# myscience/open-genie

Measured on NVIDIA H100. Metric: videotokenizer_train_step_frames_per_sec, higher is better.
Workload: dtype bf16

## Files before the change

### include/opengenie_b200.h

```cpp
#ifndef OPENGENIE_B200_H_
#define OPENGENIE_B200_H_

#include <stddef.h>
#include <stdint.h>

#ifdef __cplusplus
extern "C" {
#endif

typedef enum og_status {
  OG_OK = 0,
  OG_ERR_INVALID_ARGUMENT = -1,
  OG_ERR_UNSUPPORTED_SHAPE = -2,
  OG_ERR_CUDA = -3,
} og_status;

typedef void* og_stream_t;

const char* og_last_error(void);
int og_abi_version(void);
int og_compiled_sm(void);
uint64_t og_launch_count(void);


int og_conv3d_fwd(const void* x0, int c0, int kt, int kh, int kw, int pt, int ph, int pw, const void* x1, int c1,
                  const void* w, int ldw, const float* bias0, const float* bias1, const void* residual, void* out,
                  int out_f32, int N, int T, int H, int W, int cout, void* workspace, size_t workspace_bytes,
                  double* gn_sums, og_stream_t stream);

int og_conv3d_dgrad(const void* dy, int cout, int w_rows, const void* w, int ldw, int k_off, int kt, int kh, int kw,
                    int pt, int ph, int pw, void* dx, int dx_f32, int N, int T, int H, int W, int cin,
                    void* workspace, size_t workspace_bytes, og_stream_t stream);

int og_conv3d_wgrad(const void* dy, int cout, const void* x, int cin, float* dw, int64_t ld_dw, int kt, int kh,
                    int kw, int pt, int ph, int pw, int N, int T, int H, int W, void* workspace,
                    size_t workspace_bytes, og_stream_t stream);
int og_conv3d_wgrad_bias(const void* dy, int cout, const void* x, int cin, float* dw, int64_t ld_dw, int kt, int kh,
                         int kw, int pt, int ph, int pw, int N, int T, int H, int W, float* dbias, int n_bias,
                         void* workspace, size_t workspace_bytes, og_stream_t stream);

int og_conv3d_strided_fwd(const void* x, int cin, int kt, int kh, int kw, int st, int sh, int sw, int pt, int ph, int pw,
                          const void* w, int ldw, const float* bias, void* out, int out_f32, int N, int T, int H, int W,
                          int cout, og_stream_t stream);
int og_conv3d_strided_dgrad(const void* dy, int cout, int w_rows, const void* w, int ldw, int kt, int kh, int kw, int st,
                            int sh, int sw, int pt, int ph, int pw, void* dx, int N, int T, int H, int W, int cin,
                            og_stream_t stream);
int og_conv3d_strided_wgrad(const void* dy, int cout, const void* x, int cin, float* dw, int64_t ld_dw, int kt, int kh,
                            int kw, int st, int sh, int sw, int pt, int ph, int pw, int N, int T, int H, int W,
                            void* workspace, size_t workspace_bytes, og_stream_t stream);


int og_gn_stats(const void* x, int N, int64_t V, int C, int G, double* sums, og_stream_t stream);

int og_gn_finalize(const double* sums, int N, int C, int G, int64_t V, float eps, const float* gamma,
                   const float* beta, const float* cond_scale, const float* cond_shift, float* A, float* B,
                   float* mean_rstd, og_stream_t stream);

int og_affine_act_fwd(const void* x, const float* A, const float* B, void* y, int N, int64_t V, int C, int act,
                      og_stream_t stream);

int og_affine_act_bwd_reduce(const void* dy, const void* x, const float* A, const float* B, int act, float* S,
                             int N, int64_t V, int C, void* workspace, size_t workspace_bytes, og_stream_t stream);

int og_gn_bwd_finalize(const float* S, const float* mean_rstd, const float* gamma, const float* beta,
                       const float* cond_scale, int N, int C, int G, int64_t V, float* Q, float* R, float* dgamma,
                       float* dbeta, float* dcond_scale, float* dcond_shift, og_stream_t stream);

int og_affine_act_bwd_apply(const void* dy, const void* x, const float* A, const float* B, const float* Q,
                            const float* R, const void* add, void* dx, int act, int N, int64_t V, int C,
                            og_stream_t stream);

int og_adagn_cond_fwd(const float* cond, int N, int64_t V, int D, const float* w_scale, const float* b_scale,
                      const float* w_shift, const float* b_shift, int C, float* cbar, float* scale, float* shift,
                      og_stream_t stream);
int og_adagn_cond_bwd(const float* dscale, const float* dshift, const float* cbar, const float* w_scale,
                      const float* w_shift, int N, int64_t V, int D, int C, float* dw_scale, float* db_scale,
                      float* dw_shift, float* db_shift, float* dcond, og_stream_t stream);

int og_gn_act_fwd(const void* x, const double* sums, const float* gamma, const float* beta, const float* cond_scale,
                  const float* cond_shift, float eps, int G, int act, void* y, float* A, float* B, float* mean_rstd,
                  int N, int64_t V, int C, og_stream_t stream);
int og_gn_act_bwd(const void* dy, const void* x, const float* A, const float* B, const float* S,
                  const float* mean_rstd, const float* gamma, const float* beta, const float* cond_scale, int G, int act,
                  const void* add, void* dx, float* dgamma, float* dbeta, float* dcond_scale, float* dcond_shift,
                  float* dx_colsum, int N, int64_t V, int C, void* workspace, size_t workspace_bytes,
                  og_stream_t stream);


int og_ncdhw_f32_to_ndhwc(const float* x, void* y, int y_f32, int N, int C, int64_t V, og_stream_t stream);
int og_ndhwc_to_ncdhw_f32(const void* x, int x_f32, float* y, int N, int C, int64_t V, og_stream_t stream);

int og_pixel_shuffle3d(const void* x, void* y, int inverse, int N, int T, int H, int W, int c, int p, int q, int r,
                       og_stream_t stream);

int og_blurpool3d(const void* x, void* y, float* scratch, int backward, int N, int T, int H, int W, int cin, int cout,
                  int k, int st, int sh, int sw, og_stream_t stream);

int og_blurpool2d(const void* x, void* y, float* scratch, int backward, int N, int H, int W, int cin, int cout, int k,
                  int sh, int sw, int pad, og_stream_t stream);

int og_mse_fwd(const float* rec_ndhwc, const float* tgt_ncdhw, int N, int C, int64_t V, float* loss_sum,
               og_stream_t stream);
int og_mse_bwd(const float* rec_ndhwc, const float* tgt_ncdhw, const float* gscale, int N, int C, int cpad,
               int64_t V, void* drec, og_stream_t stream);

int og_maxpool2x2(const void* x, void* y, int N, int H, int W, int C, og_stream_t stream);
int og_sqdiff_sum(const void* a, const void* b, int64_t n, float* out, og_stream_t stream);

int og_colsum(const void* x, int64_t rows, int C, int ld, float* out, og_stream_t stream);
int og_pad_channels(const void* x, int x_f32, void* y, int64_t rows, int cs, int cd, og_stream_t stream);

int og_sub_rows(const void* a, const void* b, void* out, int64_t n, og_stream_t stream);

int og_copy_rows_to_bf16(const void* src, int src_f32, int64_t src_ld, void* dst, int64_t dst_ld, int64_t rows,
                         int cols, og_stream_t stream);

int og_frames_u8_to_video(const uint8_t* frames, int bgr, void* out, int out_kind, int cpad, int N, int T, int H, int W,
                          og_stream_t stream);

size_t og_lfq_workspace_bytes(int64_t ntok, int D);

int og_lfq_fwd(const float* x, int ldx, int64_t ntok, int D, float beta, int training, float w_commit,
               float w_entropy, float w_div, float* out_f32, void* out_bf16, int ld_bf16, int64_t* idx, float* loss,
               void* workspace, og_stream_t stream);

int og_lfq_bwd(const float* x, int ldx, int64_t ntok, int D, float beta, float w_commit, float w_entropy,
               const float* gloss, const float* dout, int ld_dout, float* dx_f32, void* dx_bf16, int ld_dx,
               void* workspace, og_stream_t stream);


int og_rope_table(const float* freq, int npos, int C, float* table, og_stream_t stream);
int og_rope_ln_fwd(const void* x, const float* freq, const float* gamma, const float* beta, float eps, void* y,
                   int64_t rows, int C, int64_t pos_div, int pos_mod, const float* cos_sin, og_stream_t stream);
int og_rope_ln_bwd(const void* x, const float* freq, const float* gamma, float eps, const void* g0, const void* g1,
                   const void* g2, const void* add, void* dx, float* dgamma, float* dbeta, int64_t rows, int C,
                   int64_t pos_div, int pos_mod, const float* cos_sin, og_stream_t stream);

int og_flash_attn_fwd(const void* q, const void* k, const void* v, void* out, const void* residual, void* out_res,
                      float* lse, int nseq, int S, int C, int n_head, float scale, og_stream_t stream);
int og_flash_attn_bwd(const void* q, const void* k, const void* v, const void* out, const void* dout,
                      const float* lse, float* delta_ws, void* dq, void* dk, void* dv, int nseq, int S, int C,
                      int n_head, float scale, og_stream_t stream);

int og_temporal_attn_fwd(const void* q, const void* k, const void* v, const void* residual, void* out, int B, int T,
                         int64_t P, int C, int n_head, float scale, int kv_bcast, og_stream_t stream);
int og_temporal_attn_bwd(const void* q, const void* k, const void* v, const void* dout, void* dq, void* dk, void* dv,
                         float* dk_bcast, float* dv_bcast, int B, int T, int64_t P, int C, int n_head, float scale,
                         int kv_bcast, og_stream_t stream);

int og_temporal_attn_long_fwd(const void* q, const void* k, const void* v, void* out, const void* residual,
                              void* out_res, float* lse, int B, int T, int64_t P, int C, int n_head, float scale,
                              int kv_bcast, og_stream_t stream);
int og_temporal_attn_long_bwd(const void* q, const void* k, const void* v, const void* out, const void* dout,
                              const float* lse, float* delta_ws, void* dq, void* dk, void* dv, float* dk_bcast,
                              float* dv_bcast, int B, int T, int64_t P, int C, int n_head, float scale, int kv_bcast,
                              og_stream_t stream);


int og_embed_add_fwd(const int64_t* tok, const int64_t* act, const float* tok_w, const float* act_w, void* out,
                     int64_t rows, int64_t rows_per_act, int C, int tok_vocab, int act_vocab, og_stream_t stream);
int og_embed_add_bwd(const int64_t* tok, const int64_t* act, const void* dy, float* d_tok_w, float* d_act_w,
                     int64_t rows, int64_t rows_per_act, int C, int tok_vocab, int act_vocab, og_stream_t stream);

int og_masked_ce_fwd(const void* logits, const int64_t* target, const uint8_t* mask, int64_t rows, int V,
                     float* row_lse, float* stats, og_stream_t stream);
int og_masked_ce_bwd(const void* logits, const int64_t* target, const uint8_t* mask, const float* row_lse,
                     const float* stats, const float* gloss, void* dlogits, int64_t rows, int V, og_stream_t stream);

int og_softmax_cdf(const void* logits, int logits_f32, int64_t rows, int V, float inv_temp, float* cdf,
                   float* row_stats, og_stream_t stream);
int og_maskgit_sample(const float* cdf, const void* logits, int logits_f32, float inv_temp, const float* row_stats,
                      const float* uniforms, const int* schedule, int steps, int B, int P, int V, int64_t* code,
                      uint8_t* mask, og_stream_t stream);

typedef struct og_adamw_tensor {
  float* p;
  const float* g;
  float* m;
  float* v;
  void* p_bf16;
  int64_t n;
  int64_t row_len;
  int64_t dst_ld;
} og_adamw_tensor;

int og_adamw_chunk_elems(void);
int og_adamw_step(const og_adamw_tensor* table_dev, const int* chunk_tensor_dev, const int* chunk_index_dev,
                  int num_chunks, float lr, float beta1, float beta2, float eps, float weight_decay, int step,
                  const int* step_dev, const float* lr_dev, const float* grad_scale_dev, og_stream_t stream);
int og_adamw_tick(int* step_dev, og_stream_t stream);

#ifdef __cplusplus
// ... 4 lines not shown
```

### open_genie_b200/csrc/conv3d_wgrad.cu

```cuda
#include "og_host.cuh"
#include "og_ptx.cuh"

namespace og {
extern std::atomic<uint64_t> g_launches;

static constexpr int kWThreads = 384;
static constexpr int kVox = 64;
static constexpr int kPanelBytes = kVox * 128;
static constexpr int kTileM = 128;
static constexpr int kTileN = 256;
static constexpr int kWABytes = 2 * kPanelBytes;
static constexpr int kWBBytes = 4 * kPanelBytes;
static constexpr int kWStages = 4;
static constexpr int kSlotFloats = kTileM * kTileN;

struct WgradParams {
  int kt, kh, kw, pt, ph, pw;
  int sx_t, sx_h, sx_w;
  int bw_log2, bh_log2, bt_log2, bn_log2;
  int tiles_w, tiles_h, tiles_t;
  int num_ksteps;
  int cin, cout;
  int ncols;
  int col_tiles;
  long long units;
  int ctas;
  int granule;
  int period;
  float* dw;
  long long ld_dw;
  int vec_ok;
  float* dbias;
  int n_bias;
  float* ws;
};

__host__ __device__ __forceinline__ long long share_begin(const WgradParams& p, int b) {
  return (long long)b * (p.units / p.granule) / p.ctas * p.granule;
}

template <bool kOnes>
__device__ __forceinline__ void wgrad_mma_steps(float (&acc)[128], float (&accb)[8], int nsteps, const uint8_t* smem_a,
                                                const uint8_t* smem_b, uint32_t ones_addr, uint64_t* full,
                                                uint64_t* empty, int& s, uint32_t& ph, int lane) {
  int prev = -1;
  for (int i = 0; i < nsteps; ++i) {
    mbar_wait(&full[s], ph);
    const uint32_t a_addr = smem_u32(smem_a + s * kWABytes);
    const uint32_t b_addr = smem_u32(smem_b + s * kWBBytes);
    wgmma_fence();
#pragma unroll
    for (int k = 0; k < kVox / 16; ++k)
      wgmma_ss<256, 1, 1>(acc, gmma_desc_sw128(a_addr + k * 2048, kPanelBytes, 1024),
                          gmma_desc_sw128(b_addr + k * 2048, kPanelBytes, 1024), (i | k) != 0);
    if constexpr (kOnes) {
#pragma unroll
      for (int k = 0; k < kVox / 16; ++k)
        wgmma_ss<16, 1, 1>(accb, gmma_desc_sw128(a_addr + k * 2048, kPanelBytes, 1024),
                           gmma_desc_sw128(ones_addr, kPanelBytes, 1024), (i | k) != 0);
    }
    wgmma_commit();
    wgmma_wait<1>();
    if (prev >= 0 && lane == 0) mbar_arrive(&empty[prev]);
    prev = s;
    if (++s == kWStages) {
      s = 0;
      ph ^= 1;
    }
  }
  wgmma_wait<0>();
  if (lane == 0) mbar_arrive(&empty[prev]);
}

template <bool kBias>
__global__ void __launch_bounds__(kWThreads, 1)
    og_conv_wgrad_kernel(const __grid_constant__ CUtensorMap mapDY, const __grid_constant__ CUtensorMap mapX,
                         const WgradParams p) {
  extern __shared__ uint8_t smem_raw[];
  uint8_t* smem = reinterpret_cast<uint8_t*>((reinterpret_cast<uintptr_t>(smem_raw) + 1023) & ~uintptr_t(1023));
  uint8_t* smem_a = smem;
  uint8_t* smem_b = smem + kWStages * kWABytes;
  uint8_t* smem_ones = smem_b + kWStages * kWBBytes;
  uint64_t* full = reinterpret_cast<uint64_t*>(smem_ones + 2048);
  uint64_t* empty = full + kWStages;

  const int warp = warp_idx_uniform();
  const int lane = threadIdx.x & 31;
  const long long u_begin = share_begin(p, blockIdx.x), u_end = share_begin(p, blockIdx.x + 1);

  if (warp == 0 && lane == 0) {
    tma_prefetch_desc(&mapDY);
    tma_prefetch_desc(&mapX);
    for (int s = 0; s < kWStages; ++s) {
      mbar_init(&full[s], 1);
      mbar_init(&empty[s], 8);
    }
    fence_mbar_init();
  }
  if (kBias) {
    for (int i = threadIdx.x; i < 2048 / 4; i += kWThreads) reinterpret_cast<uint32_t*>(smem_ones)[i] = 0x3F803F80u;
    fence_proxy_async_smem();
  }
  __syncthreads();

  if (warp == 0) {
    int s = 0;
    uint32_t ph = 0;
    const int per_sample = p.tiles_w * p.tiles_h * p.tiles_t;
    long long clock = 0;
    for (long long u = u_begin; u < u_end;) {
      const int tile = (int)(u / p.num_ksteps);
      const int k0 = (int)(u - (long long)tile * p.num_ksteps);
      const int k1 = (int)min((long long)p.num_ksteps, u_end - (long long)tile * p.num_ksteps);
      u += k1 - k0;
      const int co0 = (tile / p.col_tiles) * kTileM;
      const int c0 = (tile % p.col_tiles) * kTileN;
      const int npan = min(4, (p.ncols - c0) / 64);
      int pci[4], off_w[4], off_h[4], off_t[4];
#pragma unroll
      for (int j = 0; j < 4; ++j) {
        const int c = c0 + 64 * (j < npan ? j : 0);
        const int tap = c / p.cin;
        pci[j] = c - tap * p.cin;
        off_t[j] = tap / (p.kh * p.kw) - p.pt;
        off_h[j] = (tap / p.kw) % p.kh - p.ph;
        off_w[j] = tap % p.kw - p.pw;
      }
      const uint32_t tx_bytes = (uint32_t)(kWABytes + npan * kPanelBytes);
      int ks = k0 + (int)((clock - k0 % p.period + p.period) % p.period);
      if (ks >= k1) ks = k0;
      clock += k1 - k0;
      int tn, tw, th, tt;
      auto decode = [&](int k) {
        tn = k / per_sample;
        int r = k - tn * per_sample;
        tw = r % p.tiles_w;
        r /= p.tiles_w;
        th = r % p.tiles_h;
        tt = r / p.tiles_h;
      };
      decode(ks);
      for (int i = k0; i < k1; ++i) {
        const int n = tn << p.bn_log2, w0 = tw << p.bw_log2, h0 = th << p.bh_log2, t0 = tt << p.bt_log2;
        mbar_wait(&empty[s], ph ^ 1);
        if (elect_one()) {
          mbar_expect_tx(&full[s], tx_bytes);
          uint8_t* a = smem_a + s * kWABytes;
          tma_load_5d(a, &mapDY, &full[s], co0, w0, h0, t0, n);
          tma_load_5d(a + kPanelBytes, &mapDY, &full[s], co0 + 64, w0, h0, t0, n);
          uint8_t* b = smem_b + s * kWBBytes;
          for (int j = 0; j < npan; ++j)
            tma_load_5d(b + j * kPanelBytes, &mapX, &full[s], pci[j], w0 * p.sx_w + off_w[j], h0 * p.sx_h + off_h[j],
                        t0 * p.sx_t + off_t[j], n);
        }
        __syncwarp();
        if (++s == kWStages) {
          s = 0;
          ph ^= 1;
        }
        if (++ks == k1) {
          ks = k0;
          decode(ks);
        } else if (++tw == p.tiles_w) {
          tw = 0;
          if (++th == p.tiles_h) {
            th = 0;
            if (++tt == p.tiles_t) {
              tt = 0;
              ++tn;
            }
          }
        }
      }
    }
    __syncwarp();
  } else if (warp >= 4) {
    const int wg = (warp >> 2) - 1;
    const int q = warp & 3;
    const uint32_t ones_addr = smem_u32(smem_ones);
    const uint8_t* a_wg = smem_a + wg * kPanelBytes;
    float acc[128], accb[8];
    int s = 0;
    uint32_t ph = 0;
    for (long long u = u_begin; u < u_end;) {
      const bool first = u == u_begin;
      const int tile = (int)(u / p.num_ksteps);
      const int k0 = (int)(u - (long long)tile * p.num_ksteps);
      const int k1 = (int)min((long long)p.num_ksteps, u_end - (long long)tile * p.num_ksteps);
      u += k1 - k0;
      const int co0 = (tile / p.col_tiles) * kTileM;
      const int c0 = (tile % p.col_tiles) * kTileN;
      const bool bias_tile = kBias && c0 == 0;
      if (bias_tile)
        wgrad_mma_steps<true>(acc, accb, k1 - k0, a_wg, smem_b, ones_addr, full, empty, s, ph, lane);
      else
        wgrad_mma_steps<false>(acc, accb, k1 - k0, a_wg, smem_b, ones_addr, full, empty, s, ph, lane);
      reg_fence(acc);
      reg_fence(accb);
      const bool whole = k0 == 0 && k1 == p.num_ksteps;
      const int slot = 2 * blockIdx.x + (first ? 0 : 1);
      const int c_lane = 2 * (lane & 3);
#pragma unroll
      for (int rr = 0; rr < 2; ++rr) {
        const int r = wg * 64 + q * 16 + (lane >> 2) + rr * 8;
        const int co = co0 + r;
        if (whole) {
          if (co >= p.cout) continue;
          float* row = p.dw + (long long)co * p.ld_dw + c0 + c_lane;
#pragma unroll
          for (int j = 0; j < 32; ++j) {
            if (c0 + 8 * j + c_lane >= p.ncols) continue;
            const float v0 = acc[4 * j + 2 * rr], v1 = acc[4 * j + 2 * rr + 1];
            if (p.vec_ok) {
              float2* d = reinterpret_cast<float2*>(row + 8 * j);
              const float2 o = *d;
              *d = make_float2(o.x + v0, o.y + v1);
            } else {
              row[8 * j] += v0;
              row[8 * j + 1] += v1;
            }
          }
          if (bias_tile && (lane & 3) == 0 && co < p.n_bias) p.dbias[co] += accb[2 * rr];
        } else {
          float* sl = p.ws + ((long long)slot * kTileM + r) * kTileN + c_lane;
#pragma unroll
          for (int j = 0; j < 32; ++j)
            *reinterpret_cast<float2*>(sl + 8 * j) = make_float2(acc[4 * j + 2 * rr], acc[4 * j + 2 * rr + 1]);
          if (bias_tile && (lane & 3) == 0)
            p.ws[(long long)2 * p.ctas * kSlotFloats + (long long)slot * kTileM + r] = accb[2 * rr];
        }
      }
    }
  }
}

__global__ void __launch_bounds__(256) og_wgrad_fixup_kernel(const WgradParams p) {
  const int b = blockIdx.y;
  const long long ub = share_begin(p, b + 1);
  const int tile = (int)(ub / p.num_ksteps);
  const long long t0 = (long long)tile * p.num_ksteps, t1 = t0 + p.num_ksteps;
  if (ub == t0 || share_begin(p, b) > t0) return;
  const int co0 = (tile / p.col_tiles) * kTileM, c0 = (tile % p.col_tiles) * kTileN;
  const int e = (blockIdx.x * 256 + threadIdx.x) * 4;
  const int r = e / kTileN, c = e % kTileN;
  float4 sum = make_float4(0.f, 0.f, 0.f, 0.f);
  float sumb = 0.f;
  const bool bias = p.dbias && c0 == 0 && blockIdx.x == 0 && threadIdx.x < kTileM;
  for (int sh = b; sh < p.ctas; ++sh) {
    const long long sb = share_begin(p, sh);
    if (sb >= t1) break;
    const int slot = 2 * sh + (sb >= t0 ? 0 : 1);
    const float4 v = __ldcg(reinterpret_cast<const float4*>(p.ws + (long long)slot * kSlotFloats + e));
    sum.x += v.x;
    sum.y += v.y;
    sum.z += v.z;
    sum.w += v.w;
    if (bias) sumb += __ldcg(p.ws + (long long)2 * p.ctas * kSlotFloats + (long long)slot * kTileM + threadIdx.x);
  }
  if (co0 + r < p.cout && c0 + c < p.ncols) {
    float* d = p.dw + (long long)(co0 + r) * p.ld_dw + c0 + c;
    d[0] += sum.x;
    d[1] += sum.y;
    d[2] += sum.z;
    d[3] += sum.w;
  }
  if (bias && co0 + (int)threadIdx.x < p.n_bias) p.dbias[co0 + threadIdx.x] += sumb;
}

}

static int launch_wgrad(const void* dy, int cout, const void* x, int cin, float* dw, int64_t ld_dw, int kt, int kh, int kw,
                        int pt, int ph, int pw, int N, int T, int H, int W, int Ti, int Hi, int Wi, int st, int sh, int sw,
                        void* workspace, size_t workspace_bytes, og_stream_t stream, float* dbias = nullptr,
                        int n_bias = 0) {
  using namespace og;
  OG_REQUIRE(dy && x && dw, "conv3d_wgrad: null pointer");
  OG_REQUIRE(!dbias || (n_bias > 0 && n_bias <= cout), "conv3d_wgrad: n_bias=%d must be in 1..cout", n_bias);
  OG_REQUIRE(cin > 0 && cin % 64 == 0, "conv3d_wgrad: cin=%d must be a multiple of 64", cin);
  OG_REQUIRE(cout > 0 && cout % 8 == 0, "conv3d_wgrad: cout=%d must be a multiple of 8 (TMA row stride)", cout);
  OG_REQUIRE(kt >= 1 && kh >= 1 && kw >= 1 && pt >= 0 && ph >= 0 && pw >= 0 && pt < kt && ph < kh && pw < kw,
             "conv3d_wgrad: bad kernel/padding");
  OG_REQUIRE(st >= 1 && sh >= 1 && sw >= 1 && st <= 8 && sh <= 8 && sw <= 8, "conv3d_wgrad: bad stride");
  int bw, bh, bt, bn;
  choose_voxel_box(kVox, N, T, H, W, &bw, &bh, &bt, &bn);
  WgradParams p;
  memset(&p, 0, sizeof(p));
  p.kt = kt; p.kh = kh; p.kw = kw; p.pt = pt; p.ph = ph; p.pw = pw;
  p.sx_t = st; p.sx_h = sh; p.sx_w = sw;
  p.bw_log2 = ilog2(bw); p.bh_log2 = ilog2(bh); p.bt_log2 = ilog2(bt); p.bn_log2 = ilog2(bn);
  p.tiles_w = (W + bw - 1) / bw; p.tiles_h = (H + bh - 1) / bh; p.tiles_t = (T + bt - 1) / bt;
  p.num_ksteps = ((N + bn - 1) / bn) * p.tiles_w * p.tiles_h * p.tiles_t;
  p.cin = cin; p.cout = cout; p.dw = dw; p.ld_dw = ld_dw;
  p.ncols = kt * kh * kw * cin;
  p.col_tiles = (p.ncols + kTileN - 1) / kTileN;
  const long long tiles = (long long)((cout + kTileM - 1) / kTileM) * p.col_tiles;
  p.units = tiles * p.num_ksteps;
  const int sms = num_sms();
  p.ctas = (int)std::min<long long>(sms, std::max<long long>(1, p.units / 4));
  p.granule = 1;
  const size_t slot_bytes = (size_t)(kSlotFloats + (dbias ? kTileM : 0)) * sizeof(float);
  const long long fit = workspace ? (long long)(workspace_bytes / (2 * slot_bytes)) : 0;
  if (fit < p.ctas) {
    if (fit > tiles) {
      p.ctas = (int)fit;
    } else {
      p.granule = p.num_ksteps;
      p.ctas = (int)std::min<long long>(sms, tiles);
    }
  }
  p.period = (int)std::min<long long>(p.num_ksteps, (p.units + p.ctas - 1) / p.ctas);
  p.ws = reinterpret_cast<float*>(workspace);
  p.vec_ok = (ld_dw % 2 == 0) && ((reinterpret_cast<uintptr_t>(dw) & 7) == 0);
  p.dbias = dbias;
  p.n_bias = n_bias;
  const size_t smem_bytes = (size_t)kWStages * (kWABytes + kWBBytes) + 2048  + 1024 + 512;

  CUtensorMap mapDY, mapX;
  {
    uint64_t dims[5] = {(uint64_t)cout, (uint64_t)W, (uint64_t)H, (uint64_t)T, (uint64_t)N};
    uint64_t str[4] = {(uint64_t)cout * 2, (uint64_t)W * cout * 2, (uint64_t)H * W * cout * 2,
                       (uint64_t)T * H * W * cout * 2};
    uint32_t box[5] = {64, (uint32_t)bw, (uint32_t)bh, (uint32_t)bt, (uint32_t)bn};
    int r = make_tmap_bf16(&mapDY, dy, 5, dims, str, box);
    if (r != OG_OK) return r;
  }
  {
    uint64_t dims[5] = {(uint64_t)cin, (uint64_t)Wi, (uint64_t)Hi, (uint64_t)Ti, (uint64_t)N};
    uint64_t str[4] = {(uint64_t)cin * 2, (uint64_t)Wi * cin * 2, (uint64_t)Hi * Wi * cin * 2,
                       (uint64_t)Ti * Hi * Wi * cin * 2};
    uint32_t box[5] = {64, (uint32_t)(bw * sw), (uint32_t)(bh * sh), (uint32_t)(bt * st), (uint32_t)bn};
    uint32_t es[5] = {1, (uint32_t)sw, (uint32_t)sh, (uint32_t)st, 1};
    OG_REQUIRE(box[1] <= 256 && box[2] <= 256 && box[3] <= 256, "conv3d_wgrad: strided box exceeds the TMA limit");
    int r = make_tmap_bf16(&mapX, x, 5, dims, str, box, es);
    if (r != OG_OK) return r;
  }
  static bool attr_set = false;
  if (!attr_set) {
    OG_CHECK_CUDA(cudaFuncSetAttribute(og_conv_wgrad_kernel<false>, cudaFuncAttributeMaxDynamicSharedMemorySize,
                                       (int)smem_bytes));
    OG_CHECK_CUDA(cudaFuncSetAttribute(og_conv_wgrad_kernel<true>, cudaFuncAttributeMaxDynamicSharedMemorySize,
                                       (int)smem_bytes));
    attr_set = true;
  }
  if (dbias)
    og_conv_wgrad_kernel<true><<<p.ctas, kWThreads, smem_bytes, (cudaStream_t)stream>>>(mapDY, mapX, p);
  else
    og_conv_wgrad_kernel<false><<<p.ctas, kWThreads, smem_bytes, (cudaStream_t)stream>>>(mapDY, mapX, p);
  OG_CHECK_CUDA(cudaGetLastError());
  g_launches.fetch_add(1);
  if (p.granule == 1 && p.ctas > 1) {
    og_wgrad_fixup_kernel<<<dim3(kSlotFloats / 1024, p.ctas - 1), 256, 0, (cudaStream_t)stream>>>(p);
    OG_CHECK_CUDA(cudaGetLastError());
    g_launches.fetch_add(1);
  }
  return OG_OK;
}

extern "C" int og_conv3d_wgrad(const void* dy, int cout, const void* x, int cin, float* dw, int64_t ld_dw, int kt,
                               int kh, int kw, int pt, int ph, int pw, int N, int T, int H, int W, void* workspace,
                               size_t workspace_bytes, og_stream_t stream) {
  return launch_wgrad(dy, cout, x, cin, dw, ld_dw, kt, kh, kw, pt, ph, pw, N, T, H, W, T, H, W, 1, 1, 1, workspace,
                      workspace_bytes, stream);
}

extern "C" int og_conv3d_wgrad_bias(const void* dy, int cout, const void* x, int cin, float* dw, int64_t ld_dw, int kt,
                                    int kh, int kw, int pt, int ph, int pw, int N, int T, int H, int W, float* dbias,
                                    int n_bias, void* workspace, size_t workspace_bytes, og_stream_t stream) {
  if (!dbias) {
    og::set_error("conv3d_wgrad_bias: dbias is NULL");
    return OG_ERR_INVALID_ARGUMENT;
  }
  return launch_wgrad(dy, cout, x, cin, dw, ld_dw, kt, kh, kw, pt, ph, pw, N, T, H, W, T, H, W, 1, 1, 1, workspace,
                      workspace_bytes, stream, dbias, n_bias);
}

extern "C" int og_conv3d_strided_wgrad(const void* dy, int cout, const void* x, int cin, float* dw, int64_t ld_dw, int kt,
                                       int kh, int kw, int st, int sh, int sw, int pt, int ph, int pw, int N, int T, int H,
                                       int W, void* workspace, size_t workspace_bytes, og_stream_t stream) {
  const int To = (T + pt - kt) / st + 1, Ho = (H + 2 * ph - kh) / sh + 1, Wo = (W + 2 * pw - kw) / sw + 1;
  if (To < 1 || Ho < 1 || Wo < 1) {
    og::set_error("conv3d_strided_wgrad: empty output");
    return OG_ERR_INVALID_ARGUMENT;
  }
  return launch_wgrad(dy, cout, x, cin, dw, ld_dw, kt, kh, kw, pt, ph, pw, N, To, Ho, Wo, T, H, W, st, sh, sw, workspace,
                      workspace_bytes, stream);
}
```

### open_genie_b200/ops.py

```python
from __future__ import annotations

import ctypes
from typing import Optional, Tuple

import torch
from torch import Tensor

from . import _lib

bf16 = torch.bfloat16
f32 = torch.float32


def _stream() -> int:
    return torch.cuda.current_stream().cuda_stream


def _in_backward() -> bool:
    return torch._C._current_graph_task_id() != -1


class ZeroArena:

    SEGMENT = 256 << 20
# ... 976 lines not shown
    return y5.permute(0, 2, 3, 4, 1).reshape(rows, N)


class _EmbedAddFn(torch.autograd.Function):

    @staticmethod
    def forward(ctx, tokens, act_id, tok_w, act_w):
        _require_cuda(tok_w, 'embedding weight')
        if tokens.dim() != 4:
            raise ValueError(f'embed_add: tokens must be (B, T, H, W), got {tuple(tokens.shape)}')
        if tuple(act_id.shape) != tuple(tokens.shape[:2]):
            raise ValueError(f'embed_add: act_id shape {tuple(act_id.shape)} does not match the (B, T) = '
                             f'{tuple(tokens.shape[:2])} of the tokens (one action per token frame)')
        B, T, H, W = tokens.shape
        C = tok_w.shape[1]
        tok = tokens.detach().to(torch.int64).contiguous()
        act = act_id.detach().to(torch.int64).contiguous()
        out = torch.empty((B, T, H, W, C), dtype=bf16, device=tok_w.device)
        _lib.call('og_embed_add_fwd', tok.data_ptr(), act.data_ptr(), tok_w.data_ptr(), act_w.data_ptr(), out.data_ptr(),
                  B * T * H * W, H * W, C, tok_w.shape[0], act_w.shape[0], _stream())
        ctx.save_for_backward(tok, act)
        ctx.shapes = (tok_w.shape, act_w.shape, H * W)
        return out

    @staticmethod
    def backward(ctx, dy):
        tok, act = ctx.saved_tensors
        ts, as_, hw = ctx.shapes
        dy = _rows_bf16(dy)
        dtw = _zeros(ts, f32, dy.device)
        daw = _zeros(as_, f32, dy.device)
        _lib.call('og_embed_add_bwd', tok.data_ptr(), act.data_ptr(), dy.data_ptr(), dtw.data_ptr(), daw.data_ptr(),
                  tok.numel(), hw, ts[1], ts[0], as_[0], _stream())
        return None, None, dtw, daw


def embed_add(tokens, act_id, tok_w, act_w):
    return _EmbedAddFn.apply(tokens, act_id, tok_w, act_w)


class _MaskedCeFn(torch.autograd.Function):

    @staticmethod
    def forward(ctx, logits2d, target, mask):
        rows, V = logits2d.shape
        lg = logits2d if (logits2d.dtype == bf16 and logits2d.is_contiguous()) else logits2d.to(bf16).contiguous()
        tgt = target.detach().reshape(-1).to(torch.int64).contiguous()
        msk = mask.detach().reshape(-1).to(torch.uint8).contiguous()
        row_lse = torch.empty(rows, dtype=f32, device=lg.device)
        stats = torch.zeros(2, dtype=f32, device=lg.device)
        _lib.call('og_masked_ce_fwd', lg.data_ptr(), tgt.data_ptr(), msk.data_ptr(), rows, V, row_lse.data_ptr(),
                  stats.data_ptr(), _stream())
        ctx.save_for_backward(lg, tgt, msk, row_lse, stats)
        return stats[0] / stats[1]

    @staticmethod
    def backward(ctx, g):
        lg, tgt, msk, row_lse, stats = ctx.saved_tensors
        gs = g.detach().to(f32).contiguous()
        dl = torch.empty_like(lg)
        _lib.call('og_masked_ce_bwd', lg.data_ptr(), tgt.data_ptr(), msk.data_ptr(), row_lse.data_ptr(), stats.data_ptr(),
                  gs.data_ptr(), dl.data_ptr(), lg.shape[0], lg.shape[1], _stream())
        return dl, None, None


def masked_cross_entropy(logits2d, target, mask):
    return _MaskedCeFn.apply(logits2d, target, mask)


def maskgit_sample(logits_last: Tensor, uniforms: Tensor, schedule: Tensor, temp: float = 1.0, masked_tok: int = 0
                   ) -> Tensor:
    _require_cuda(logits_last, 'logits')
    b, h, w, V = logits_last.shape
    P = h * w
    lg = logits_last.detach()
    if lg.dtype not in (bf16, f32) or not lg.is_contiguous():
        lg = lg.float().contiguous()
    dev = lg.device
    s = _stream()
    cdf = torch.empty((b * P, V), dtype=f32, device=dev)
    row_stats = torch.empty((b * P, 2), dtype=f32, device=dev)
    lg_f32, inv_temp = int(lg.dtype == f32), 1.0 / float(temp)
    _lib.call('og_softmax_cdf', lg.data_ptr(), lg_f32, b * P, V, inv_temp, cdf.data_ptr(), row_stats.data_ptr(), s)
    steps = int(schedule.numel())
    u = uniforms.detach().to(device=dev, dtype=f32).reshape(steps, b * P).contiguous()
    sch = schedule.detach().to(device=dev, dtype=torch.int32).contiguous()
    code = torch.full((b, P), int(masked_tok), dtype=torch.int64, device=dev)
    mask = torch.ones((b, P), dtype=torch.uint8, device=dev)
    _lib.call('og_maskgit_sample', cdf.data_ptr(), lg.data_ptr(), lg_f32, inv_temp, row_stats.data_ptr(), u.data_ptr(),
              sch.data_ptr(), steps, b, P, V, code.data_ptr(), mask.data_ptr(), s)
    return code.view(b, h, w), mask.view(b, h, w)


class _ResBlockFn(torch.autograd.Function):

    @staticmethod
    def forward(ctx, x, x_sums, g1w, g1b, w1, b1, g2w, g2b, w2, b2, wres, bres, packed1, packed2, geom1: ConvGeom,
                geom2: ConvGeom, G: int, eps: float, act: int = 1):
        _require_cuda(x, 'residual block input')
        xi = to_internal(x, bf16)
        B, C0, T, H, W = xi.shape
        C1 = geom1.cout
        V = T * H * W
        s = _stream()
        dev = xi.device
        rec = any(ctx.needs_input_grad)
        if x_sums is None:
            x_sums = _zeros((B, G, 2), torch.float64, dev, rec)
            _lib.call('og_gn_stats', xi.data_ptr(), B, V, C0, G, x_sums.data_ptr(), s)
        mr = torch.empty((2, B, G, 2), dtype=f32, device=dev)
        A1, B1 = torch.empty((B, C0), dtype=f32, device=dev), torch.empty((B, C0), dtype=f32, device=dev)
        A2, B2 = torch.empty((B, C1), dtype=f32, device=dev), torch.empty((B, C1), dtype=f32, device=dev)
        a1 = empty_internal(B, C0, T, H, W, bf16, dev)
        _lib.call('og_gn_act_fwd', xi.data_ptr(), x_sums.data_ptr(), g1w.data_ptr(), g1b.data_ptr(), None, None, eps, G, act,
                  a1.data_ptr(), A1.data_ptr(), B1.data_ptr(), mr[0].data_ptr(), B, V, C0, s)
        ws = _workspace(dev, B * V * C1 * 4)
        fuse_stats = G == 1
        sums2 = _zeros((B, G, 2), torch.float64, dev, rec)
        h1 = empty_internal(B, C1, T, H, W, bf16, dev)
        _conv_call('fwd', 2.0 * B * V * C1 * geom1.k_main, 'og_conv3d_fwd', a1.data_ptr(), C0, geom1.kt, geom1.kh,
                   geom1.kw, geom1.pt, geom1.ph, geom1.pw, None, 0, packed1.data_ptr(), packed1.shape[1], _ptr(b1), None,
                   None, h1.data_ptr(), 0, B, T, H, W, C1, ws.data_ptr(), ws.numel(),
                   sums2.data_ptr() if fuse_stats else None, s)
        if not fuse_stats:
            _lib.call('og_gn_stats', h1.data_ptr(), B, V, C1, G, sums2.data_ptr(), s)
        a2 = empty_internal(B, C1, T, H, W, bf16, dev)
        _lib.call('og_gn_act_fwd', h1.data_ptr(), sums2.data_ptr(), g2w.data_ptr(), g2b.data_ptr(), None, None, eps, G, act,
                  a2.data_ptr(), A2.data_ptr(), B2.data_ptr(), mr[1].data_ptr(), B, V, C1, s)
        y = empty_internal(B, C1, T, H, W, bf16, dev)
        y_sums = _zeros((B, 1, 2), torch.float64, dev, rec)
        _conv_call('fwd', 2.0 * B * V * C1 * (geom2.k_main + C0), 'og_conv3d_fwd', a2.data_ptr(), C1, geom2.kt, geom2.kh,
                   geom2.kw, geom2.pt, geom2.ph, geom2.pw, xi.data_ptr(), C0, packed2.data_ptr(), packed2.shape[1],
                   _ptr(b2), _ptr(bres), None, y.data_ptr(), 0, B, T, H, W, C1, ws.data_ptr(), ws.numel(),
                   y_sums.data_ptr(), s)
        ctx.cfg = (geom1, geom2, G, b1 is not None, b2 is not None, bres is not None, act)
        ctx.save_for_backward(xi, a1, h1, a2, A1, B1, A2, B2, mr, g1w, g1b, g2w, g2b, packed1, packed2)
        ctx.mark_non_differentiable(y_sums)
        ctx.set_materialize_grads(False)
        return y, y_sums

    @staticmethod
    def backward(ctx, dy, _dsums):
        xi, a1, h1, a2, A1, B1, A2, B2, mr, g1w, g1b, g2w, g2b, packed1, packed2 = ctx.saved_tensors
        geom1, geom2, G, has_b1, has_b2, has_bres, act = ctx.cfg
        B, C0, T, H, W = xi.shape
        C1 = geom1.cout
        V = T * H * W
        s = _stream()
        dev = xi.device
        dyb = _as_bf16_rows(dy, C1, C1)
        ws = _workspace(dev, B * V * max(C0, C1) * 4)
        ld2 = packed2.shape[1]

        def wgrad(dyt, cout, xin, cin, g, dbias=None):
            gr = _zeros((cout, g.ntaps * cin), f32, dev)
            if dbias is None:
                _conv_call('wgrad', 2.0 * B * V * cout * cin * g.ntaps, 'og_conv3d_wgrad', dyt.data_ptr(), cout,
                           xin.data_ptr(), cin, gr.data_ptr(), gr.shape[1], g.kt, g.kh, g.kw, g.pt, g.ph, g.pw, B, T, H, W,
                           *_scratch(dyt), s)
            else:
                _conv_call('wgrad', 2.0 * B * V * cout * cin * g.ntaps, 'og_conv3d_wgrad_bias', dyt.data_ptr(), cout,
                           xin.data_ptr(), cin, gr.data_ptr(), gr.shape[1], g.kt, g.kh, g.kw, g.pt, g.ph, g.pw, B, T, H, W,
                           dbias.data_ptr(), cout, *_scratch(dyt), s)
            return gr.view(cout, g.kt, g.kh, g.kw, cin).permute(0, 4, 1, 2, 3)

        gone = ConvGeom(C0, C1, (1, 1, 1))
        db2 = _zeros(C1, f32, dev)
        dw2 = wgrad(dyb, C1, a2, C1, geom2)
        dwres = wgrad(dyb, C1, xi, C0, gone, dbias=db2)
        S2 = _zeros((B, C1, 2), f32, dev)
        d_a2 = empty_internal(B, C1, T, H, W, bf16, dev)
        _conv_call('dgrad', 2.0 * B * V * C1 * geom2.k_main, 'og_conv3d_dgrad', dyb.data_ptr(), C1, C1, packed2.data_ptr(),
                   ld2, 0, geom2.kt, geom2.kh, geom2.kw, geom2.pt, geom2.ph, geom2.pw, d_a2.data_ptr(), 0, B, T, H, W, C1,
                   ws.data_ptr(), ws.numel(), s)
        small = _zeros((3, C1), f32, dev)
        dg2w, dg2b, db1 = small[0], small[1], small[2]
        d_h1 = empty_internal(B, C1, T, H, W, bf16, dev)
        _gn_bwd(d_a2, h1, A2, B2, S2, mr[1], g2w, g2b, G, act, None, d_h1, dg2w, dg2b, db1 if has_b1 else None, B, V, C1, s)
        dw1 = wgrad(d_h1, C1, a1, C0, geom1)
        dx = None
        dg1w, dg1b = _zeros(C0, f32, dev), _zeros(C0, f32, dev)
        dx_res = empty_internal(B, C0, T, H, W, bf16, dev)
        S1 = _zeros((B, C0, 2), f32, dev)
        d_a1 = empty_internal(B, C0, T, H, W, bf16, dev)
        _conv_call('dgrad', 2.0 * B * V * C1 * geom1.k_main, 'og_conv3d_dgrad', d_h1.data_ptr(), C1, C1,
                   packed1.data_ptr(), packed1.shape[1], 0, geom1.kt, geom1.kh, geom1.kw, geom1.pt, geom1.ph, geom1.pw,
                   d_a1.data_ptr(), 0, B, T, H, W, C0, ws.data_ptr(), ws.numel(), s)
        _lib.call('og_affine_act_bwd_reduce', d_a1.data_ptr(), xi.data_ptr(), A1.data_ptr(), B1.data_ptr(), act,
                  S1.data_ptr(), B, V, C0, *_scratch(d_a1), s)
        _conv_call('dgrad', 2.0 * B * V * C1 * C0, 'og_conv3d_dgrad', dyb.data_ptr(), C1, C1, packed2.data_ptr(), ld2,
                   geom2.k_main, 1, 1, 1, 0, 0, 0, dx_res.data_ptr(), 0, B, T, H, W, C0, ws.data_ptr(), ws.numel(), s)
        dx = empty_internal(B, C0, T, H, W, bf16, dev)
        _gn_bwd(d_a1, xi, A1, B1, S1, mr[0], g1w, g1b, G, act, dx_res, dx, dg1w, dg1b, None, B, V, C0, s, reduce=False)
        return (dx, None, dg1w, dg1b, dw1, db1 if has_b1 else None, dg2w, dg2b, dw2, db2 if has_b2 else None, dwres,
                (db2.clone() if has_b2 else db2) if has_bres else None, None, None, None, None, None, None, None)


def residual_block(x, x_sums, g1w, g1b, w1, b1, g2w, g2b, w2, b2, wres, bres, packed1, packed2, geom1, geom2, G, eps,
                   act='silu'):
    return _ResBlockFn.apply(x, x_sums, g1w, g1b, w1, b1, g2w, g2b, w2, b2, wres, bres, packed1, packed2, geom1, geom2, G,
                             float(eps), act_code(act))
```

Baseline: 1040.

## Fuse shortcut 1x1 wgrad into main conv wgrad as extra GEMM columns

Adds a wgrad entry point that appends the residual-shortcut input channels as extra column panels, loaded through a second TMA map, so the main 3D conv weight gradient and the 1x1 shortcut weight gradient come from one kernel pass over dy. This removes a separate launch and a second full read of dy. The kernel also skips the upper 64-row dy load and MMA work when cout does not fill the 128-row tile. In exchange, the epilogue and column bookkeeping gain extra branching, and the tile and load-balancing layout shifts.

```diff
diff --git a/include/opengenie_b200.h b/include/opengenie_b200.h
--- a/include/opengenie_b200.h
+++ b/include/opengenie_b200.h
@@ -38,6 +38,10 @@
 int og_conv3d_wgrad_bias(const void* dy, int cout, const void* x, int cin, float* dw, int64_t ld_dw, int kt, int kh,
                          int kw, int pt, int ph, int pw, int N, int T, int H, int W, float* dbias, int n_bias,
                          void* workspace, size_t workspace_bytes, og_stream_t stream);
+int og_conv3d_wgrad_shortcut(const void* dy, int cout, const void* x, int cin, float* dw, int64_t ld_dw, int kt,
+                             int kh, int kw, int pt, int ph, int pw, const void* x_sc, int cin_sc, float* dw_sc,
+                             int64_t ld_dw_sc, float* dbias, int n_bias, int N, int T, int H, int W,
+                             void* workspace, size_t workspace_bytes, og_stream_t stream);
 
 int og_conv3d_strided_fwd(const void* x, int cin, int kt, int kh, int kw, int st, int sh, int sw, int pt, int ph, int pw,
                           const void* w, int ldw, const float* bias, void* out, int out_f32, int N, int T, int H, int W,
diff --git a/open_genie_b200/csrc/conv3d_wgrad.cu b/open_genie_b200/csrc/conv3d_wgrad.cu
--- a/open_genie_b200/csrc/conv3d_wgrad.cu
+++ b/open_genie_b200/csrc/conv3d_wgrad.cu
@@ -21,6 +21,7 @@
   int tiles_w, tiles_h, tiles_t;
   int num_ksteps;
   int cin, cout;
+  int ncols_main;
   int ncols;
   int col_tiles;
   long long units;
@@ -29,11 +30,18 @@
   int period;
   float* dw;
   long long ld_dw;
+  float* dw_sc;
+  long long ld_dw_sc;
   int vec_ok;
   float* dbias;
   int n_bias;
   float* ws;
 };
+
+__device__ __forceinline__ float* dw_at(const WgradParams& p, int co, int c) {
+  return c < p.ncols_main ? p.dw + (long long)co * p.ld_dw + c
+                          : p.dw_sc + (long long)co * p.ld_dw_sc + (c - p.ncols_main);
+}
 
 __host__ __device__ __forceinline__ long long share_begin(const WgradParams& p, int b) {
   return (long long)b * (p.units / p.granule) / p.ctas * p.granule;
@@ -75,7 +83,7 @@
 template <bool kBias>
 __global__ void __launch_bounds__(kWThreads, 1)
     og_conv_wgrad_kernel(const __grid_constant__ CUtensorMap mapDY, const __grid_constant__ CUtensorMap mapX,
-                         const WgradParams p) {
+                         const __grid_constant__ CUtensorMap mapXsc, const WgradParams p) {
   extern __shared__ uint8_t smem_raw[];
   uint8_t* smem = reinterpret_cast<uint8_t*>((reinterpret_cast<uintptr_t>(smem_raw) + 1023) & ~uintptr_t(1023));
   uint8_t* smem_a = smem;
@@ -91,6 +99,7 @@
   if (warp == 0 && lane == 0) {
     tma_prefetch_desc(&mapDY);
     tma_prefetch_desc(&mapX);
+    if (p.ncols > p.ncols_main) tma_prefetch_desc(&mapXsc);
     for (int s = 0; s < kWStages; ++s) {
       mbar_init(&full[s], 1);
       mbar_init(&empty[s], 8);
@@ -117,16 +126,25 @@
       const int c0 = (tile % p.col_tiles) * kTileN;
       const int npan = min(4, (p.ncols - c0) / 64);
       int pci[4], off_w[4], off_h[4], off_t[4];
+      const CUtensorMap* pmap[4];
 #pragma unroll
       for (int j = 0; j < 4; ++j) {
         const int c = c0 + 64 * (j < npan ? j : 0);
+        if (c >= p.ncols_main) {
+          pmap[j] = &mapXsc;
+          pci[j] = c - p.ncols_main;
+          off_t[j] = off_h[j] = off_w[j] = 0;
+          continue;
+        }
         const int tap = c / p.cin;
+        pmap[j] = &mapX;
         pci[j] = c - tap * p.cin;
         off_t[j] = tap / (p.kh * p.kw) - p.pt;
         off_h[j] = (tap / p.kw) % p.kh - p.ph;
         off_w[j] = tap % p.kw - p.pw;
       }
-      const uint32_t tx_bytes = (uint32_t)(kWABytes + npan * kPanelBytes);
+      const bool rows_hi = co0 + 64 < p.cout;
+      const uint32_t tx_bytes = (uint32_t)((rows_hi ? kWABytes : kPanelBytes) + npan * kPanelBytes);
       int ks = k0 + (int)((clock - k0 % p.period + p.period) % p.period);
       if (ks >= k1) ks = k0;
       clock += k1 - k0;
@@ -147,10 +165,10 @@
           mbar_expect_tx(&full[s], tx_bytes);
           uint8_t* a = smem_a + s * kWABytes;
           tma_load_5d(a, &mapDY, &full[s], co0, w0, h0, t0, n);
-          tma_load_5d(a + kPanelBytes, &mapDY, &full[s], co0 + 64, w0, h0, t0, n);
+          if (rows_hi) tma_load_5d(a + kPanelBytes, &mapDY, &full[s], co0 + 64, w0, h0, t0, n);
           uint8_t* b = smem_b + s * kWBBytes;
           for (int j = 0; j < npan; ++j)
-            tma_load_5d(b + j * kPanelBytes, &mapX, &full[s], pci[j], w0 * p.sx_w + off_w[j], h0 * p.sx_h + off_h[j],
+            tma_load_5d(b + j * kPanelBytes, pmap[j], &full[s], pci[j], w0 * p.sx_w + off_w[j], h0 * p.sx_h + off_h[j],
                         t0 * p.sx_t + off_t[j], n);
         }
         __syncwarp();
@@ -191,6 +209,17 @@
       const int co0 = (tile / p.col_tiles) * kTileM;
       const int c0 = (tile % p.col_tiles) * kTileN;
       const bool bias_tile = kBias && c0 == 0;
+      if (co0 + 64 * wg >= p.cout) {
+        for (int i = k0; i < k1; ++i) {
+          mbar_wait(&full[s], ph);
+          if (lane == 0) mbar_arrive(&empty[s]);
+          if (++s == kWStages) {
+            s = 0;
+            ph ^= 1;
+          }
+        }
+        continue;
+      }
       if (bias_tile)
         wgrad_mma_steps<true>(acc, accb, k1 - k0, a_wg, smem_b, ones_addr, full, empty, s, ph, lane);
       else
@@ -207,17 +236,19 @@
         if (whole) {
           if (co >= p.cout) continue;
           float* row = p.dw + (long long)co * p.ld_dw + c0 + c_lane;
+          float* row_sc = p.dw_sc + (long long)co * p.ld_dw_sc + (c0 - p.ncols_main) + c_lane;
 #pragma unroll
           for (int j = 0; j < 32; ++j) {
             if (c0 + 8 * j + c_lane >= p.ncols) continue;
+            float* d = (c0 + 8 * j < p.ncols_main ? row : row_sc) + 8 * j;
             const float v0 = acc[4 * j + 2 * rr], v1 = acc[4 * j + 2 * rr + 1];
             if (p.vec_ok) {
-              float2* d = reinterpret_cast<float2*>(row + 8 * j);
-              const float2 o = *d;
-              *d = make_float2(o.x + v0, o.y + v1);
+              float2* d2 = reinterpret_cast<float2*>(d);
+              const float2 o = *d2;
+              *d2 = make_float2(o.x + v0, o.y + v1);
             } else {
-              row[8 * j] += v0;
-              row[8 * j + 1] += v1;
+              d[0] += v0;
+              d[1] += v1;
             }
           }
           if (bias_tile && (lane & 3) == 0 && co < p.n_bias) p.dbias[co] += accb[2 * rr];
@@ -258,7 +289,7 @@
     if (bias) sumb += __ldcg(p.ws + (long long)2 * p.ctas * kSlotFloats + (long long)slot * kTileM + threadIdx.x);
   }
   if (co0 + r < p.cout && c0 + c < p.ncols) {
-    float* d = p.dw + (long long)(co0 + r) * p.ld_dw + c0 + c;
+    float* d = dw_at(p, co0 + r, c0 + c);
     d[0] += sum.x;
     d[1] += sum.y;
     d[2] += sum.z;
@@ -272,11 +303,15 @@
 static int launch_wgrad(const void* dy, int cout, const void* x, int cin, float* dw, int64_t ld_dw, int kt, int kh, int kw,
                         int pt, int ph, int pw, int N, int T, int H, int W, int Ti, int Hi, int Wi, int st, int sh, int sw,
                         void* workspace, size_t workspace_bytes, og_stream_t stream, float* dbias = nullptr,
-                        int n_bias = 0) {
+                        int n_bias = 0, const void* x_sc = nullptr, int cin_sc = 0, float* dw_sc = nullptr,
+                        int64_t ld_dw_sc = 0) {
   using namespace og;
   OG_REQUIRE(dy && x && dw, "conv3d_wgrad: null pointer");
   OG_REQUIRE(!dbias || (n_bias > 0 && n_bias <= cout), "conv3d_wgrad: n_bias=%d must be in 1..cout", n_bias);
   OG_REQUIRE(cin > 0 && cin % 64 == 0, "conv3d_wgrad: cin=%d must be a multiple of 64", cin);
+  OG_REQUIRE(cin_sc == 0 || (x_sc && dw_sc && cin_sc % 64 == 0 && ld_dw_sc >= cin_sc),
+             "conv3d_wgrad_shortcut: x_sc and dw_sc must be non-null, cin_sc=%d a multiple of 64, ld_dw_sc >= cin_sc",
+             cin_sc);
   OG_REQUIRE(cout > 0 && cout % 8 == 0, "conv3d_wgrad: cout=%d must be a multiple of 8 (TMA row stride)", cout);
   OG_REQUIRE(kt >= 1 && kh >= 1 && kw >= 1 && pt >= 0 && ph >= 0 && pw >= 0 && pt < kt && ph < kh && pw < kw,
              "conv3d_wgrad: bad kernel/padding");
@@ -291,7 +326,9 @@
   p.tiles_w = (W + bw - 1) / bw; p.tiles_h = (H + bh - 1) / bh; p.tiles_t = (T + bt - 1) / bt;
   p.num_ksteps = ((N + bn - 1) / bn) * p.tiles_w * p.tiles_h * p.tiles_t;
   p.cin = cin; p.cout = cout; p.dw = dw; p.ld_dw = ld_dw;
-  p.ncols = kt * kh * kw * cin;
+  p.dw_sc = dw_sc; p.ld_dw_sc = ld_dw_sc;
+  p.ncols_main = kt * kh * kw * cin;
+  p.ncols = p.ncols_main + cin_sc;
   p.col_tiles = (p.ncols + kTileN - 1) / kTileN;
   const long long tiles = (long long)((cout + kTileM - 1) / kTileM) * p.col_tiles;
   p.units = tiles * p.num_ksteps;
@@ -310,7 +347,8 @@
   }
   p.period = (int)std::min<long long>(p.num_ksteps, (p.units + p.ctas - 1) / p.ctas);
   p.ws = reinterpret_cast<float*>(workspace);
-  p.vec_ok = (ld_dw % 2 == 0) && ((reinterpret_cast<uintptr_t>(dw) & 7) == 0);
+  p.vec_ok = (ld_dw % 2 == 0) && ((reinterpret_cast<uintptr_t>(dw) & 7) == 0) &&
+             (!cin_sc || ((ld_dw_sc % 2 == 0) && ((reinterpret_cast<uintptr_t>(dw_sc) & 7) == 0)));
   p.dbias = dbias;
   p.n_bias = n_bias;
   const size_t smem_bytes = (size_t)kWStages * (kWABytes + kWBBytes) + 2048  + 1024 + 512;
@@ -334,6 +372,16 @@
     int r = make_tmap_bf16(&mapX, x, 5, dims, str, box, es);
     if (r != OG_OK) return r;
   }
+  CUtensorMap mapXsc = mapX;
+  if (cin_sc) {
+    OG_REQUIRE(st == 1 && sh == 1 && sw == 1, "conv3d_wgrad_shortcut: stride-1 convolutions only");
+    uint64_t dims[5] = {(uint64_t)cin_sc, (uint64_t)W, (uint64_t)H, (uint64_t)T, (uint64_t)N};
+    uint64_t str[4] = {(uint64_t)cin_sc * 2, (uint64_t)W * cin_sc * 2, (uint64_t)H * W * cin_sc * 2,
+                       (uint64_t)T * H * W * cin_sc * 2};
+    uint32_t box[5] = {64, (uint32_t)bw, (uint32_t)bh, (uint32_t)bt, (uint32_t)bn};
+    int r = make_tmap_bf16(&mapXsc, x_sc, 5, dims, str, box);
+    if (r != OG_OK) return r;
+  }
   static bool attr_set = false;
   if (!attr_set) {
     OG_CHECK_CUDA(cudaFuncSetAttribute(og_conv_wgrad_kernel<false>, cudaFuncAttributeMaxDynamicSharedMemorySize,
@@ -343,9 +391,9 @@
     attr_set = true;
   }
   if (dbias)
-    og_conv_wgrad_kernel<true><<<p.ctas, kWThreads, smem_bytes, (cudaStream_t)stream>>>(mapDY, mapX, p);
+    og_conv_wgrad_kernel<true><<<p.ctas, kWThreads, smem_bytes, (cudaStream_t)stream>>>(mapDY, mapX, mapXsc, p);
   else
-    og_conv_wgrad_kernel<false><<<p.ctas, kWThreads, smem_bytes, (cudaStream_t)stream>>>(mapDY, mapX, p);
+    og_conv_wgrad_kernel<false><<<p.ctas, kWThreads, smem_bytes, (cudaStream_t)stream>>>(mapDY, mapX, mapXsc, p);
   OG_CHECK_CUDA(cudaGetLastError());
   g_launches.fetch_add(1);
   if (p.granule == 1 && p.ctas > 1) {
@@ -372,6 +420,18 @@
   }
   return launch_wgrad(dy, cout, x, cin, dw, ld_dw, kt, kh, kw, pt, ph, pw, N, T, H, W, T, H, W, 1, 1, 1, workspace,
                       workspace_bytes, stream, dbias, n_bias);
+}
+
+extern "C" int og_conv3d_wgrad_shortcut(const void* dy, int cout, const void* x, int cin, float* dw, int64_t ld_dw,
+                                        int kt, int kh, int kw, int pt, int ph, int pw, const void* x_sc, int cin_sc,
+                                        float* dw_sc, int64_t ld_dw_sc, float* dbias, int n_bias, int N, int T, int H,
+                                        int W, void* workspace, size_t workspace_bytes, og_stream_t stream) {
+  if (cin_sc <= 0) {
+    og::set_error("conv3d_wgrad_shortcut: cin_sc=%d must be positive", cin_sc);
+    return OG_ERR_INVALID_ARGUMENT;
+  }
+  return launch_wgrad(dy, cout, x, cin, dw, ld_dw, kt, kh, kw, pt, ph, pw, N, T, H, W, T, H, W, 1, 1, 1, workspace,
+                      workspace_bytes, stream, dbias, dbias ? n_bias : 0, x_sc, cin_sc, dw_sc, ld_dw_sc);
 }
 
 extern "C" int og_conv3d_strided_wgrad(const void* dy, int cout, const void* x, int cin, float* dw, int64_t ld_dw, int kt,
diff --git a/open_genie_b200/ops.py b/open_genie_b200/ops.py
--- a/open_genie_b200/ops.py
+++ b/open_genie_b200/ops.py
@@ -1152,22 +1152,15 @@
         ws = _workspace(dev, B * V * max(C0, C1) * 4)
         ld2 = packed2.shape[1]
 
-        def wgrad(dyt, cout, xin, cin, g, dbias=None):
-            gr = _zeros((cout, g.ntaps * cin), f32, dev)
-            if dbias is None:
-                _conv_call('wgrad', 2.0 * B * V * cout * cin * g.ntaps, 'og_conv3d_wgrad', dyt.data_ptr(), cout,
-                           xin.data_ptr(), cin, gr.data_ptr(), gr.shape[1], g.kt, g.kh, g.kw, g.pt, g.ph, g.pw, B, T, H, W,
-                           *_scratch(dyt), s)
-            else:
-                _conv_call('wgrad', 2.0 * B * V * cout * cin * g.ntaps, 'og_conv3d_wgrad_bias', dyt.data_ptr(), cout,
-                           xin.data_ptr(), cin, gr.data_ptr(), gr.shape[1], g.kt, g.kh, g.kw, g.pt, g.ph, g.pw, B, T, H, W,
-                           dbias.data_ptr(), cout, *_scratch(dyt), s)
-            return gr.view(cout, g.kt, g.kh, g.kw, cin).permute(0, 4, 1, 2, 3)
-
-        gone = ConvGeom(C0, C1, (1, 1, 1))
+        def as_weight(gr, kt, kh, kw, cin):
+            return gr.view(gr.shape[0], kt, kh, kw, cin).permute(0, 4, 1, 2, 3)
+
         db2 = _zeros(C1, f32, dev)
-        dw2 = wgrad(dyb, C1, a2, C1, geom2)
-        dwres = wgrad(dyb, C1, xi, C0, gone, dbias=db2)
+        gr2, grres = _zeros((C1, geom2.ntaps * C1), f32, dev), _zeros((C1, C0), f32, dev)
+        _conv_call('wgrad', 2.0 * B * V * C1 * (geom2.k_main + C0), 'og_conv3d_wgrad_shortcut', dyb.data_ptr(), C1,
+                   a2.data_ptr(), C1, gr2.data_ptr(), gr2.shape[1], geom2.kt, geom2.kh, geom2.kw, geom2.pt, geom2.ph,
+                   geom2.pw, xi.data_ptr(), C0, grres.data_ptr(), C0, db2.data_ptr(), C1, B, T, H, W, *_scratch(dyb), s)
+        dw2, dwres = as_weight(gr2, geom2.kt, geom2.kh, geom2.kw, C1), as_weight(grres, 1, 1, 1, C0)
         S2 = _zeros((B, C1, 2), f32, dev)
         d_a2 = empty_internal(B, C1, T, H, W, bf16, dev)
         _conv_call('dgrad', 2.0 * B * V * C1 * geom2.k_main, 'og_conv3d_dgrad', dyb.data_ptr(), C1, C1, packed2.data_ptr(),
@@ -1177,7 +1170,11 @@
         dg2w, dg2b, db1 = small[0], small[1], small[2]
         d_h1 = empty_internal(B, C1, T, H, W, bf16, dev)
         _gn_bwd(d_a2, h1, A2, B2, S2, mr[1], g2w, g2b, G, act, None, d_h1, dg2w, dg2b, db1 if has_b1 else None, B, V, C1, s)
-        dw1 = wgrad(d_h1, C1, a1, C0, geom1)
+        gr1 = _zeros((C1, geom1.ntaps * C0), f32, dev)
+        _conv_call('wgrad', 2.0 * B * V * C1 * geom1.k_main, 'og_conv3d_wgrad', d_h1.data_ptr(), C1, a1.data_ptr(), C0,
+                   gr1.data_ptr(), gr1.shape[1], geom1.kt, geom1.kh, geom1.kw, geom1.pt, geom1.ph, geom1.pw, B, T, H, W,
+                   *_scratch(d_h1), s)
+        dw1 = as_weight(gr1, geom1.kt, geom1.kh, geom1.kw, C0)
         dx = None
         dg1w, dg1b = _zeros(C0, f32, dev), _zeros(C0, f32, dev)
         dx_res = empty_internal(B, C0, T, H, W, bf16, dev)
```

Result: no change. 1049 (median of 6 runs) (+0.8%).
